# adamnelsonarcher/BB-OCR

Measured on AMD Instinct MI355X. Metric: book-page images/sec end-to-end (detect+recognize) @1280x960, higher is better.
Workload: dtype fp16

## Files before the change

### bb-ocr_amd/csrc/abi.cpp

```cpp
#include "ctx.h"

static hipError_t create_seq_stream(hipStream_t* s) {
    return hipStreamCreateWithFlags(s, hipStreamNonBlocking);
}

extern "C" {

void bbocr_default_params(bbocr_params* p) {
    if (!p) return;
    memset(p, 0, sizeof(*p));
    p->text_threshold = 0.7; p->low_text = 0.4; p->link_threshold = 0.4; p->canvas_size = 2560; p->mag_ratio = 1.0;
    p->slope_ths = 0.1; p->ycenter_ths = 0.5; p->height_ths = 0.5; p->width_ths = 0.5; p->add_margin = 0.1; p->min_size = 20;
    p->contrast_ths = 0.1; p->adjust_contrast = 0.5;
    p->decoder = BBOCR_DECODER_GREEDY; p->beam_width = 5;
}

int bbocr_create(const bbocr_config* cfg, bbocr_ctx** out) {
    if (!out) return BBOCR_ERR_ARG;
    *out = nullptr;
    bbocr_ctx* c = nullptr;
    try {
        c = new bbocr_ctx();
        c->root = c;
        if (cfg) c->cfg = *cfg;
        if (c->cfg.precision < BBOCR_PREC_BF16 || c->cfg.precision > BBOCR_PREC_EXACT_REC || c->cfg.call_slots < 0 || c->cfg.call_slots > kMaxSlots ||
            c->cfg.rec_quant < 0 || c->cfg.rec_quant > 1 || (c->cfg.rec_quant == 1 && !rec_split(c))) {
            delete c;
            return BBOCR_ERR_ARG;
        }
        int ndev = 0;
        if (hipGetDeviceCount(&ndev) != hipSuccess || ndev <= 0 || c->cfg.device < 0 || c->cfg.device >= ndev) {
            delete c;
            return BBOCR_ERR_HIP;
        }
        if (hipSetDevice(c->cfg.device) != hipSuccess || hipStreamCreateWithFlags(&c->stream, hipStreamNonBlocking) != hipSuccess ||
            hipStreamCreateWithFlags(&c->stream2, hipStreamNonBlocking) != hipSuccess ||
            create_seq_stream(&c->seq_stream) != hipSuccess ||
            hipMalloc(&c->zero_page, 256) != hipSuccess || hipMemset(c->zero_page, 0, 256) != hipSuccess) {
            delete c;
            return BBOCR_ERR_HIP;
        }
    } catch (...) {
        delete c;
        return BBOCR_ERR_INTERNAL;
    }
    c->cur = c->stream;
    *out = c;
    return BBOCR_OK;
}

}

bbocr_ctx* slot_create(bbocr_ctx* root) {
    bbocr_ctx* s = new bbocr_ctx();
    s->root = root;
    s->cfg = root->cfg;
    s->stream = root->stream;
    hipError_t e = hipStreamCreateWithFlags(&s->stream2, hipStreamNonBlocking);
    if (e == hipSuccess) e = create_seq_stream(&s->seq_stream);
    if (e != hipSuccess) {
        if (s->stream2) (void)hipStreamDestroy(s->stream2);
        delete s;
        fail(BBOCR_ERR_HIP, std::string("call slot: ") + hipGetErrorString(e));
    }
    s->cur = s->stream;
    return s;
}

void slot_destroy(bbocr_ctx* c) {
    if (c->stream2) (void)hipStreamSynchronize(c->stream2);
    if (c->seq_stream) (void)hipStreamSynchronize(c->seq_stream);
    if (c->feat_ev) (void)hipEventDestroy(c->feat_ev);
    for (hipEvent_t e : c->sub_events) (void)hipEventDestroy(e);
    if (c->det_t0) { (void)hipEventDestroy(c->det_t0); (void)hipEventDestroy(c->det_t1); }
    if (c->ccl_t0) { (void)hipEventDestroy(c->ccl_t0); (void)hipEventDestroy(c->ccl_t1); }
    if (c->sync_ev) (void)hipEventDestroy(c->sync_ev);
    if (c->seq_t1) { (void)hipEventDestroy(c->seq_t1); (void)hipEventDestroy(c->seq_t2); }
    for (auto& r : c->prof_recs) { (void)hipEventDestroy(r.e0); (void)hipEventDestroy(r.e1); }
    for (hipEvent_t e : c->prof_pool) (void)hipEventDestroy(e);
    DevBuf* bufs[] = {&c->arena.buf, &c->heat, &c->gray, &c->resized, &c->ccl_label, &c->ccl_stat, &c->ccl_slot, &c->ccl_comps, &c->ccl_rowext,
                      &c->ccl_counters, &c->crop_desc, &c->crop_desc2, &c->crop_scratch, &c->crop_hscratch, &c->crop_wscratch, &c->crop_luts, &c->crop_hist,
                      &c->ctc_idx, &c->ctc_pmax, &c->ctc_out_idx, &c->ctc_out, &c->seq_v, &c->seq_xp, &c->seq_h, &c->seq_lin, &c->seq_logits,
                      &c->seq_tables, &c->pp_gray, &c->pp_a, &c->pp_b, &c->pp_c, &c->pp_tab, &c->ctc_probs, &c->ctc_beam_idx, &c->ctc_beam_len, &c->ac_work, &c->th_coef, &c->je_scan, &c->je_out, &c->pe_out,
                      &c->pg_rgb, &c->pg_tab, &c->seq_q8, &c->seq_rowp};
    for (DevBuf* b : bufs) b->release();
    if (c->stream2) (void)hipStreamDestroy(c->stream2);
    if (c->seq_stream) (void)hipStreamDestroy(c->seq_stream);
    if (c->root != c) delete c;
}

namespace {
struct ThreadTimes { const bbocr_ctx* root = nullptr; float ms[8] = {0}; };
thread_local ThreadTimes tl_times;
thread_local std::string tl_err;
}
void publish_times(const bbocr_ctx* s) {
    tl_times.root = s->root;
    memcpy(tl_times.ms, s->times, sizeof(tl_times.ms));
}

extern "C" {

void bbocr_destroy(bbocr_ctx* c) {
    if (!c) return;
    (void)hipSetDevice(c->cfg.device);
    if (c->stream) (void)hipStreamSynchronize(c->stream);
    dist_release(c);
    for (bbocr_ctx* s : c->slots) slot_destroy(s);
    c->slots.clear();
    free_weights(c);
    slot_destroy(c);
    if (c->zero_page) (void)hipFree(c->zero_page);
    for (SideLane* l : {&c->upload_lane, &c->jpeg_lane})
        if (l->stream) (void)hipStreamDestroy(l->stream);
    if (c->stream) (void)hipStreamDestroy(c->stream);
    delete c;
}

const char* bbocr_last_error(bbocr_ctx* c) {
    if (!c) return "null context";
    std::lock_guard<std::mutex> lk(c->pool_mu);
    tl_err = c->err;
    return tl_err.c_str();
}

// ... 62 lines not shown
        detect_impl(ctx, dev_rgb, B, H, W, pp, dev_heat_out);
        slot_sync(ctx, ctx->stream);
        prof_collect(ctx);
        ctx->times[0] = ctx->times[7] = (float)ms_since(t0);
    });
}

int bbocr_boxes(bbocr_ctx* ctx, const float* dev_heat, int B, int h, int w, double ratio, const bbocr_params* p, bbocr_boxlist** out) {
    return guarded(ctx, [&](bbocr_ctx* ctx) {
        bbocr_params pp;
        bbocr_default_params(&pp);
        if (p) pp = *p;
        if (!dev_heat || !out) fail(BBOCR_ERR_ARG, "null pointer");
        memset(ctx->times, 0, sizeof(ctx->times));
        auto t0 = clk::now();
        HostBoxes hb;
        boxes_impl(ctx, dev_heat, B, h, w, ratio, pp, hb, ctx->stream);
        *out = export_boxes(hb);
        ctx->times[7] = (float)ms_since(t0);
    });
}

int bbocr_recognize(bbocr_ctx* ctx, const uint8_t* dev_gray, int B, int H, int W, const bbocr_boxlist* boxes, const bbocr_params* p,
                    bbocr_result** out) {
    return guarded(ctx, [&](bbocr_ctx* ctx) {
        bbocr_params pp;
        bbocr_default_params(&pp);
        if (p) pp = *p;
        if (!dev_gray || !boxes || !out || boxes->n_images != B) fail(BBOCR_ERR_ARG, "bad recognise arguments");
        memset(ctx->times, 0, sizeof(ctx->times));
        auto t0 = clk::now();
        HostBoxes hb;
        import_boxes(boxes, hb);
        std::vector<BoxJob> jobs;
        std::vector<int> off;
        recognize_impl(ctx, GrayPages{dev_gray, H, W}, B, hb, pp, jobs, off);
        prof_collect(ctx);
        *out = export_result(B, jobs, off);
        ctx->times[7] = (float)ms_since(t0);
    });
}

int bbocr_readtext_batch(bbocr_ctx* ctx, const uint8_t* dev_rgb, const uint8_t* dev_gray, int B, int H, int W, const bbocr_params* p,
                         bbocr_result** out) {
    return guarded(ctx, [&](bbocr_ctx* ctx) {
        bbocr_params pp;
        bbocr_default_params(&pp);
        if (p) pp = *p;
        if (!dev_rgb || !out) fail(BBOCR_ERR_ARG, "null pointer");
        memset(ctx->times, 0, sizeof(ctx->times));
        auto t_all = clk::now();
        const DetDims d = det_dims(H, W, pp.canvas_size, pp.mag_ratio);
        ctx->heat.ensure((size_t)B * d.h * d.w * 2 * sizeof(float));
        if (!dev_gray) {
            ctx->gray.ensure((size_t)B * H * W);
            HIPCHK(launch_gray(dev_rgb, (uint8_t*)ctx->gray.p, (size_t)B * H * W, ctx->stream));
            dev_gray = (const uint8_t*)ctx->gray.p;
        }
        std::vector<std::pair<int, int>> subs;
        if (!ctx->det_t0) { HIPCHK(hipEventCreate(&ctx->det_t0)); HIPCHK(hipEventCreate(&ctx->det_t1)); }
        HIPCHK(hipEventRecord(ctx->det_t0, ctx->stream));
        detect_impl(ctx, dev_rgb, B, H, W, pp, (float*)ctx->heat.p, [&](int b0, int nb) {
            if (subs.size() >= ctx->sub_events.size()) {
                hipEvent_t e;
                HIPCHK(hipEventCreateWithFlags(&e, hipEventDisableTiming));
                ctx->sub_events.push_back(e);
            }
            HIPCHK(hipEventRecord(ctx->sub_events[subs.size()], ctx->stream));
            subs.push_back({b0, nb});
        });
        HIPCHK(hipEventRecord(ctx->det_t1, ctx->stream));
        HostBoxes hb;
        hb.polys.resize(B); hb.hori.resize(B); hb.freeb.resize(B);
        RecEarly early;
        for (size_t k = 0; k < subs.size(); ++k) {
            const int b0 = subs[k].first, nb = subs[k].second;
            HIPCHK(hipStreamWaitEvent(ctx->stream2, ctx->sub_events[k], 0));
            HostBoxes part;
            boxes_impl(ctx, (const float*)ctx->heat.p + (size_t)b0 * d.h * d.w * 2, nb, d.h, d.w, d.ratio, pp, part, ctx->stream2);
            for (int i = 0; i < nb; ++i) {
                hb.polys[b0 + i] = std::move(part.polys[i]);
                hb.hori[b0 + i] = std::move(part.hori[i]);
                hb.freeb[b0 + i] = std::move(part.freeb[i]);
            }
            if (subs.size() >= 2 && k + 2 == subs.size() && pp.rotation_info[0] == 0 && ctx->crnn_loaded)
                rec_early_begin(ctx, GrayPages{dev_gray, H, W}, b0 + nb, B, hb, pp, early);
        }
        HIPCHK(hipEventSynchronize(ctx->det_t1));
        float det_ms = 0.f;
        HIPCHK(hipEventElapsedTime(&det_ms, ctx->det_t0, ctx->det_t1));
        ctx->times[0] = det_ms;
        std::vector<BoxJob> jobs;
        std::vector<int> off;
        recognize_impl(ctx, GrayPages{dev_gray, H, W}, B, hb, pp, jobs, off, &early);
        prof_collect(ctx);
        *out = export_result(B, jobs, off);
        ctx->times[7] = (float)ms_since(t_all);
    });
}

void bbocr_preproc_defaults(bbocr_preproc_params* p, int legacy) {
    if (!p) return;
    memset(p, 0, sizeof(*p));
    p->scale = 1.5; p->unsharp_radius = 1.0; p->unsharp_threshold = 3;
    if (legacy) { p->blur_sigma = 5.0; p->contrast = 1.3; p->brightness = 0.0; p->clahe_clip = 2.0; p->unsharp_percent = 20; }
    else        { p->blur_sigma = 3.0; p->contrast = 1.9; p->brightness = 1.2; p->clahe_clip = 2.5; p->unsharp_percent = 30; }
}

int bbocr_preprocess_chain(bbocr_ctx* ctx, const uint8_t* dev_bgr, int H, int W, const bbocr_preproc_params* p, uint8_t* dev_out, int* out_h,
                           int* out_w) {
    return guarded(ctx, [&](bbocr_ctx* ctx) {
        bbocr_preproc_params q;
        bbocr_preproc_defaults(&q, 0);
        if (p) q = *p;
        if (H <= 0 || W <= 0) fail(BBOCR_ERR_ARG, "bad image shape");
        if (q.scale < 0 || q.blur_sigma < 0 || q.contrast < 0 || q.brightness < 0 || q.clahe_clip < 0 || q.unsharp_radius < 0 || q.unsharp_percent < 0)
            fail(BBOCR_ERR_ARG, "negative pre-processing parameter");
        const int dh = q.scale > 0 ? (int)(H * q.scale) : H, dw = q.scale > 0 ? (int)(W * q.scale) : W;
        if (out_h) *out_h = dh;
        if (out_w) *out_w = dw;
        if (!dev_out) return;
        if (!dev_bgr) fail(BBOCR_ERR_ARG, "null device pointer");
        if (dh <= 0 || dw <= 0) fail(BBOCR_ERR_ARG, "image collapses to zero size");
        if (q.clahe_clip > 0 && (dh < 16 || dw < 16)) fail(BBOCR_ERR_ARG, "image too small for the 8x8 CLAHE tile grid");
        preprocess_chain_impl(ctx, dev_bgr, H, W, q, dev_out, dh, dw);
    });
}

int bbocr_preprocess_book_cover(bbocr_ctx* ctx, const uint8_t* dev_bgr, int H, int W, uint8_t* dev_out, int* out_h, int* out_w) {
    bbocr_preproc_params q;
    bbocr_preproc_defaults(&q, 0);
    return bbocr_preprocess_chain(ctx, dev_bgr, H, W, &q, dev_out, out_h, out_w);
}

void bbocr_free_boxlist(bbocr_boxlist* b) {
    if (!b) return;
    free(b->poly_off); free(b->polys); free(b->hori_off); free(b->hori); free(b->free_off); free(b->free_q);
    free(b);
}

void bbocr_free_result(bbocr_result* r) {
    if (!r) return;
    free(r->box_off); free(r->quads); free(r->is_free); free(r->text_off); free(r->text_idx); free(r->conf);
    free(r);
}

int bbocr_set_profiling(bbocr_ctx* ctx, int on) {
// ... 25 lines not shown
```

### bb-ocr_amd/csrc/ctx.h

```cpp
#pragma once
#include "../../include/bbocr.h"

#include <algorithm>
#include <atomic>
#include <chrono>
#include <condition_variable>
#include <cmath>
#include <cstring>
#include <functional>
#include <map>
#include <memory>
#include <mutex>
#include <string>
#include <thread>
#include <unordered_map>
#include <vector>

#include "boxpost.h"
#include "hostpool.h"
#include "common.h"
#include "kernels.h"


using clk = std::chrono::steady_clock;
// ... 112 lines not shown
    bool craft_loaded = false;
    uint16_t* c11_wf = nullptr;
    float* c11_b = nullptr;
    float* c11_w32 = nullptr;
    float* cls6_w32 = nullptr;
    ConvPlan conv1_2, conv2_1, conv2_2, conv3_1, conv3_2, conv3_3, conv4_1, conv4_2, conv4_3, conv5_1, conv5_2, fc6, fc7;
    ConvPlan up1a, up1b, up2b, up3b, up4b, cls0, cls2, cls4;
    ConvPlan up2y, up2s, up3y, up3s, up4y, up4s;
    float* cls_tail = nullptr;
    uint16_t* cls_tail_frag = nullptr;
    uint16_t* up4y_post = nullptr;
    bool crnn_loaded = false;
    float* r0_wb = nullptr;
    uint16_t* r0_afrag = nullptr;
    ConvPlan r1, r2, r3, r4, r5, r6, xproj[2], lin[2], pred;
    uint16_t* whh[2] = {nullptr, nullptr};
    float whh_scale[2] = {1.f, 1.f};
    struct Q8Layer { int8_t* w = nullptr; float* scale = nullptr; float* bias = nullptr; };
    Q8Layer q_ih[2], q_hh[2], q_lin[2], q_pred;
    void* zero_page = nullptr;
};

struct bbocr_ctx : WeightView {
    bbocr_config cfg{};
    bbocr_ctx* root = nullptr;
    std::vector<bbocr_ctx*> slots;
    std::mutex pool_mu;
    std::condition_variable pool_cv;
    std::mutex enq_mu;
    ConvRoute op_conv_route{};
    bool slot_busy = false;
    hipStream_t stream = nullptr;
    DevBuf pp_gray, pp_a, pp_b, pp_c, pp_tab;
    DevBuf ac_work;
    DevBuf th_coef;
    int th_coef_key[6] = {0, 0, 0, 0, 0, 0};
    int th_coef_ks[2] = {0, 0};
    int th_coef_rows[2] = {0, 0};
    DevBuf je_scan, je_out;
    DevBuf pe_out;
    DevBuf pp_cubic;
    int pp_cubic_key[4] = {0, 0, 0, 0};
    unsigned long long pp_cubic_K[2] = {0, 0};
    unsigned int ignore_mask[4] = {0, 0, 0, 0};
    int beam_width = 0;
    hipStream_t cur = nullptr;
    SideLane upload_lane;
    SideLane jpeg_lane;
    PinBuf jd_pin;
    DevBuf jd_in, jd_work, jd_coef, jd_stage;
    DevBuf jd_page;
    long long jd_count[4] = {0, 0, 0, 0};
    hipStream_t seq_stream = nullptr;
    hipEvent_t feat_ev = nullptr;
    hipStream_t stream2 = nullptr;
    std::vector<hipEvent_t> sub_events;
    hipEvent_t ccl_t0 = nullptr, ccl_t1 = nullptr;
    hipEvent_t det_t0 = nullptr, det_t1 = nullptr;
    hipEvent_t sync_ev = nullptr;
    hipEvent_t seq_t1 = nullptr, seq_t2 = nullptr;
    std::string err;
    float times[8] = {0};

    struct ProfRec { hipEvent_t e0, e1; double flops; int group; };
    int profiling = 0;
    int prof_group = 0;
    std::vector<ProfRec> prof_recs;
    std::vector<hipEvent_t> prof_pool;
    double prof_ms[2] = {0, 0}, prof_flops[2] = {0, 0};
    long long prof_launches[2] = {0, 0};

    void* dist_comm = nullptr;
    int dist_rank = 0, dist_world = 0;
    std::unique_ptr<HostPool> pool;
    std::vector<void*> owned;
    std::vector<size_t> owned_bytes;

    Arena arena;
    DevBuf heat, gray, resized;
    DevBuf pg_rgb, pg_tab;
    PinBuf pg_pin;
    DevBuf ccl_label, ccl_stat, ccl_slot, ccl_comps, ccl_rowext, ccl_counters;
    DevBuf crop_desc, crop_scratch, crop_hscratch, crop_wscratch, crop_luts, crop_hist;
    DevBuf ctc_idx, ctc_pmax, ctc_out_idx, ctc_out, ctc_probs, ctc_beam_idx, ctc_beam_len, crop_desc2;
    PinBuf desc_pin, desc_pin2;
    PinBuf ctc_pin;
    DevBuf seq_v, seq_xp, seq_h, seq_lin, seq_logits, seq_tables;
    DevBuf seq_q8, seq_rowp;
};

inline int det_el(const bbocr_ctx* c) { return (c->cfg.precision == BBOCR_PREC_FP16 || c->cfg.precision == BBOCR_PREC_EXACT || c->cfg.precision == BBOCR_PREC_EXACT_REC) ? 1 : 0; }
inline int rec_el(const bbocr_ctx* c) { return c->cfg.precision != BBOCR_PREC_BF16 ? 1 : 0; }
inline bool rec_split(const bbocr_ctx* c) { return c->cfg.precision == BBOCR_PREC_EXACT || c->cfg.precision == BBOCR_PREC_EXACT_REC; }
inline bool rec_quant(const bbocr_ctx* c) { return c->cfg.rec_quant == 1; }
inline bool det_split(const bbocr_ctx* c) { return c->cfg.precision == BBOCR_PREC_EXACT; }

struct TensorMap {
    std::unordered_map<std::string, const bbocr_tensor_desc*> m;
    bool zeros = false;
    std::vector<float> zero_buf;
    TensorMap() : zeros(true), zero_buf((size_t)5 << 20, 0.f) {}
    TensorMap(const bbocr_tensor_desc* d, int n) {
        for (int i = 0; i < n; ++i) {
            std::string k = d[i].name ? d[i].name : "";
            if (k.rfind("module.", 0) == 0) k = k.substr(7);
            m[k] = &d[i];
        }
// ... 160 lines not shown
void crnn_seq_xproj(bbocr_ctx* c, int l, const uint16_t* x, size_t rows_pad, void* xp);
void crnn_seq_xproj_conv(bbocr_ctx* c, int l, const uint16_t* x, size_t rows_pad, void* xp);
void crnn_seq_lin(bbocr_ctx* c, int l, const uint16_t* h, size_t rows_pad, uint16_t* out);
void crnn_seq_pred(bbocr_ctx* c, const uint16_t* x, size_t rows_pad, float* logits);
void rec_seq_tiles(const bbocr_ctx* c, RecRun& run);
enum { CTC_GREEDY = 0, CTC_BEAM_HOST = 1, CTC_BEAM_DEVICE = 2 };
int ctc_route(int beam_width, int C, const int* seqs, int nseq);
void ctc_size(bbocr_ctx* c, size_t rows, int nseq, int cs, int route);
double ctc_decode(const CtcOut& o, const int* idx, int n, std::vector<int>& text);
void rec_early_begin(bbocr_ctx* c, const GrayPages& g, int pages, int B, const HostBoxes& hb, const bbocr_params& p, RecEarly& e);
void recognize_impl(bbocr_ctx* c, const GrayPages& g, int B, const HostBoxes& hb, const bbocr_params& p, std::vector<BoxJob>& jobs, std::vector<int>& box_off, RecEarly* early = nullptr);
bbocr_result* export_result(int B, const std::vector<BoxJob>& jobs, const std::vector<int>& box_off);
void pp_resize(bbocr_ctx* c, const uint8_t* src, int H, int W, uint8_t* dst, int dh, int dw, bool src_bgr = false);
void pp_gauss(bbocr_ctx* c, const uint8_t* src, int H, int W, uint8_t* dst, double sigma);
const uint8_t* pp_fold_lut(bbocr_ctx* c, size_t n, double contrast, double brightness);
void pp_clahe(bbocr_ctx* c, const uint8_t* src, int H, int W, const uint8_t* d_lut, uint8_t* dst, double clip_limit);
void pp_unsharp(bbocr_ctx* c, const uint8_t* src, int H, int W, uint8_t* dst, uint8_t* tmp1, uint8_t* tmp2, float radius, int percent, int threshold);
void preprocess_chain_impl(bbocr_ctx* c, const uint8_t* bgr, int H, int W, const bbocr_preproc_params& q, uint8_t* out, int dh, int dw);
void gaussian_taps_fixed(int n, double sigma, int* k);

inline HostPool& host_pool(bbocr_ctx* c) {
    if (!c->pool) {
        const int want = c->cfg.host_threads > 0 ? c->cfg.host_threads : std::min(16, host_cpu_share());
        c->pool.reset(new HostPool(std::max(1, std::min(want, 64)) - 1));
    }
    return *c->pool;
}

inline bool other_call_in_flight(bbocr_ctx* c) {
    bbocr_ctx* root = c->root;
    std::lock_guard<std::mutex> lk(root->pool_mu);
    if (root != c && root->slot_busy) return true;
    for (bbocr_ctx* s : root->slots)
        if (s != c && s->slot_busy) return true;
    return false;
}

struct EnqLock {
    std::unique_lock<std::mutex> lk;
    explicit EnqLock(bbocr_ctx* c) : lk(c->root->enq_mu) {}
};
constexpr int kMaxSlots = 2;
bbocr_ctx* slot_create(bbocr_ctx* root);
void slot_destroy(bbocr_ctx* s);
void publish_times(const bbocr_ctx* s);
void dist_release(bbocr_ctx* root);

inline void slot_sync(bbocr_ctx* c, hipStream_t st) {
    if (!c->sync_ev) HIPCHK(hipEventCreateWithFlags(&c->sync_ev, hipEventDisableTiming));
    HIPCHK(hipEventRecord(c->sync_ev, st));
    HIPCHK(hipEventSynchronize(c->sync_ev));
}

inline void prof_release(bbocr_ctx* c, const bbocr_ctx::ProfRec& r) { c->prof_pool.push_back(r.e0); c->prof_pool.push_back(r.e1); }

inline void guarded_drain(bbocr_ctx* ctx) {
    if (ctx->stream) (void)hipStreamSynchronize(ctx->stream);
    if (ctx->stream2) (void)hipStreamSynchronize(ctx->stream2);
    if (ctx->seq_stream) (void)hipStreamSynchronize(ctx->seq_stream);
    ctx->cur = ctx->stream;
    (void)hipGetLastError();
    for (auto& r : ctx->prof_recs) prof_release(ctx, r);
    ctx->prof_recs.clear();
}

struct SlotLease {
    bbocr_ctx* root;
    bbocr_ctx* slot = nullptr;
    bool exclusive;
    SlotLease(bbocr_ctx* r, bool excl) : root(r), exclusive(excl) {
        std::unique_lock<std::mutex> lk(root->pool_mu);
        const int max_slots = root->cfg.call_slots == 1 ? 1 : kMaxSlots;
        if (exclusive) {
            root->pool_cv.wait(lk, [&] {
                if (root->slot_busy) return false;
                for (bbocr_ctx* s : root->slots) if (s->slot_busy) return false;
                return true;
            });
            root->slot_busy = true;
            for (bbocr_ctx* s : root->slots) s->slot_busy = true;
            slot = root;
            return;
        }
        for (;;) {
            if (!root->slot_busy) { slot = root; break; }
            for (bbocr_ctx* s : root->slots) if (!s->slot_busy) { slot = s; break; }
            if (slot) break;
            if ((int)root->slots.size() + 1 < max_slots) {
                slot = slot_create(root);
                root->slots.push_back(slot);
                break;
            }
            root->pool_cv.wait(lk);
        }
        slot->slot_busy = true;
        if (slot != root) {
            static_cast<WeightView&>(*slot) = static_cast<const WeightView&>(*root);
            slot->cfg = root->cfg;
            slot->profiling = root->profiling;
        }
    }
    ~SlotLease() {
        {
            std::lock_guard<std::mutex> lk(root->pool_mu);
            if (exclusive) {
                root->slot_busy = false;
// ... 65 lines not shown
```

### bb-ocr_amd/csrc/recognizer.cpp

```cpp
#include "ctx.h"

void crop_refit_fw(CropDesc& d) {
    const int cw = (int)std::ceil(64 * ((double)d.rw / (double)d.rh));
    d.fw = cw > d.imgW ? d.imgW : cw;
}

static bool plan_sizes(CropDesc& d, int width, int height) {
    double ratio = (double)width / (double)height;
    if (ratio < 1.0) {
        ratio = 1.0 / ratio;
        d.rw = 64; d.rh = (int)(64 * ratio);
    } else {
        d.rw = (int)(64 * ratio); d.rh = 64;
    }
    if ((int)(64 * ratio) == 0) return false;
    d.imgW = (int)std::ceil(std::max(ratio, 1.0)) * 64;
    crop_refit_fw(d);
    return d.rw > 0 && d.rh > 0 && d.fw > 0;
}

bool plan_horizontal(const std::array<int, 4>& box, int img, int H, int W, BoxJob& j) {
    const int x_min = std::max(0, box[0]), x_max = std::min(box[1], W), y_min = std::max(0, box[2]), y_max = std::min(box[3], H);
    const int width = x_max - x_min, height = y_max - y_min;
    if (width <= 0 || height <= 0) return false;
// ... 137 lines not shown

static Act seq_rows(const bbocr_ctx* c, const uint16_t* p, size_t rows_pad, int C) { return Act{(uint16_t*)p, 1, (int)(rows_pad / 256), 256, C * rec_mul(c)}; }
void crnn_seq_xproj_conv(bbocr_ctx* c, int l, const uint16_t* x, size_t rows_pad, void* xp) {
    run_conv(c, c->xproj[l], seq_rows(c, x, rows_pad, 256), false, nullptr, false, false, xp, 2048, 2048, rec_split(c));
}
void crnn_seq_xproj(bbocr_ctx* c, int l, const uint16_t* x, size_t rows_pad, void* xp) {
    if (!rec_split(c)) {
        if (c->arena.dry) return;
        if (launch_seq_proj_profiled(c, c->xproj[l], x, rows_pad, (uint16_t*)xp) == hipSuccess) return;
    }
    crnn_seq_xproj_conv(c, l, x, rows_pad, xp);
}
void crnn_seq_lin(bbocr_ctx* c, int l, const uint16_t* h, size_t rows_pad, uint16_t* out) {
    run_conv(c, c->lin[l], seq_rows(c, h, rows_pad, 512), false, nullptr, false, false, out, 256 * rec_mul(c), 256, false);
}
void crnn_seq_pred(bbocr_ctx* c, const uint16_t* x, size_t rows_pad, float* logits) {
    run_conv(c, c->pred, seq_rows(c, x, rows_pad, 256), false, nullptr, false, false, logits, 112, 112, true);
}

static size_t rec_max_rows(const bbocr_ctx* c) { return c->cfg.rec_max_cols > 0 ? (size_t)std::max(64, c->cfg.rec_max_cols / 4) : (size_t)1500000; }

void rec_plan_part(const std::vector<BoxJob>& jobs, const std::vector<int>& sel, int res0, size_t row_base, RecPart& part) {
    std::map<int, std::vector<int>> buckets;
    for (size_t k = 0; k < sel.size(); ++k) buckets[jobs[sel[k]].d.imgW].push_back((int)k);
    size_t rows = row_base, cols = 0;
    for (auto& kv : buckets) {
        const int imgW = kv.first, T = imgW / 4 - 1;
        RecChunk ch{imgW, T, (int)part.descs.size(), (int)kv.second.size(), rows};
        for (int i = 0; i < ch.n; ++i) {
            const int k = kv.second[i];
            CropDesc d = jobs[sel[k]].d;
            if (cols > 0x7ff00000u) fail(BBOCR_ERR_OVERFLOW, "recogniser pass wider than 2^31 columns");
            d.slot = (int)cols;
            d.pad_ = (int)(rows + (size_t)i * T);
            cols += (size_t)imgW + REC_GAP;
            part.any_warp |= d.warp != 0;
            part.any_tall |= !(d.fw == d.rw && d.rh == 64);
            part.descs.push_back(d);
            part.order.push_back(res0 + k);
        }
        rows += (size_t)ch.n * T;
        part.chunks.push_back(ch);
    }
    part.rows = rows - row_base;
    part.cols = cols;
}

const CropDesc* rec_upload_descs(bbocr_ctx* c, const RecPart& part, DevBuf& desc_buf) {
    const size_t bytes = part.descs.size() * sizeof(CropDesc);
    desc_buf.ensure(bytes);
    PinBuf& pin = (&desc_buf == &c->crop_desc2) ? c->desc_pin2 : c->desc_pin;
    pin.ensure(bytes);
    memcpy(pin.p, part.descs.data(), bytes);
    HIPCHK(hipMemcpyAsync(desc_buf.p, pin.p, bytes, hipMemcpyHostToDevice, c->stream));
    return (const CropDesc*)desc_buf.p;
}

uint16_t* rec_wide_image(bbocr_ctx* c, const RecPart& part) {
    c->arena.begin(true);
    (void)c->arena.alloc<uint16_t>((size_t)64 * part.cols);
    crnn_features_wide(c, part, nullptr, nullptr);
    c->arena.buf.ensure(c->arena.off);
    c->arena.begin(false);
    return c->arena.alloc<uint16_t>((size_t)64 * part.cols);
}

void rec_launch_crops(bbocr_ctx* c, const GrayPages& g, const RecPart& part, const CropDesc* dd, uint16_t* wide, int stage) {
    const int n = (int)part.descs.size(), Wt = (int)part.cols;
    HIPCHK(launch_crops(g.gray, g.H, g.W, dd, 0, n, 0, part.any_warp, part.any_tall, (uint8_t*)c->crop_wscratch.p, (uint8_t*)c->crop_scratch.p,
                        (uint8_t*)c->crop_hscratch.p, (const uint8_t*)c->crop_luts.p, wide, stage, c->stream, wide ? Wt : 0, wide ? REC_GAP : 0,
                        wide ? rec_mode(c) : 0, g.tab_dev));
}

static void rec_launch_part(bbocr_ctx* c, const GrayPages& g, const RecPart& part, DevBuf& desc_buf, bool stage_a) {
    if (part.descs.empty()) return;
    EnqLock enq(c);
    const CropDesc* dd = rec_upload_descs(c, part, desc_buf);
    if (stage_a) rec_launch_crops(c, g, part, dd, nullptr, 1);
    uint16_t* wide = rec_wide_image(c, part);
    rec_launch_crops(c, g, part, dd, wide, 2);
    crnn_features_wide(c, part, dd, wide);
    if (!c->feat_ev) HIPCHK(hipEventCreateWithFlags(&c->feat_ev, hipEventDisableTiming));
    HIPCHK(hipEventRecord(c->feat_ev, c->stream));
}

void rec_add_tables(RecRun& run, const RecPart& part, int tile_seqs) {
    for (const RecChunk& ch : part.chunks) {
        for (int s0 = 0; s0 < ch.n; s0 += tile_seqs) {
            run.tiles.push_back((int)(ch.row0 + (size_t)s0 * ch.T));
            run.tiles.push_back(std::min(tile_seqs, ch.n - s0));
            run.tiles.push_back(ch.T);
            run.tiles.push_back(0);
        }
        for (int i = 0; i < ch.n; ++i) {
            run.seqs.push_back((int)(ch.row0 + (size_t)i * ch.T));
            run.seqs.push_back(ch.T);
            run.seq_k.push_back(part.order[ch.first + i]);
        }
    }
    run.rows += part.rows;
}

int ctc_route(int beam_width, int C, const int* seqs, int nseq) {
    if (beam_width <= 0) return CTC_GREEDY;
    int max_T = 0;
    for (int i = 0; i < nseq; ++i) max_T = std::max(max_T, seqs[2 * i + 1]);
    return ctc_beam_on_device(beam_width, C, max_T) ? CTC_BEAM_DEVICE : CTC_BEAM_HOST;
}

void ctc_size(bbocr_ctx* c, size_t rows, int nseq, int cs, int route) {
    c->ctc_idx.ensure(rows * 4);
    c->ctc_pmax.ensure(rows * 4);
    c->ctc_out_idx.ensure(rows * 4);
    c->ctc_out.ensure((size_t)nseq * sizeof(CtcOut));
    if (route != CTC_GREEDY) c->ctc_probs.ensure(rows * cs * sizeof(float));
    if (route == CTC_BEAM_DEVICE) {
        c->ctc_beam_idx.ensure(rows * 4);
        c->ctc_beam_len.ensure((size_t)nseq * 4);
    }
}

double ctc_decode(const CtcOut& o, const int* idx, int n, std::vector<int>& text) {
    text.assign(idx, idx + n);
    return o.cnt > 0 ? std::pow((double)o.prod, 2.0 / std::sqrt((double)o.cnt)) : 0.0;
}

static void rec_finish(bbocr_ctx* c, RecRun& run, std::vector<std::vector<int>>& texts, std::vector<double>& confs) {
    const size_t rows = run.rows;
    if (rows == 0) return;
    const size_t rows_pad = align_up(rows, 256);
    auto t0 = clk::now();
    rec_seq_tiles(c, run);
    {
        std::vector<int>& tiles = run.tiles;
        const size_t nt = tiles.size() / 4;
        std::vector<size_t> perm(nt);
        for (size_t i = 0; i < nt; ++i) perm[i] = i;
        std::stable_sort(perm.begin(), perm.end(), [&](size_t x, size_t y) { return tiles[x * 4 + 2] > tiles[y * 4 + 2]; });
        std::vector<int> t2(tiles.size());
        for (size_t i = 0; i < nt; ++i) memcpy(&t2[i * 4], &tiles[perm[i] * 4], 16);
        tiles.swap(t2);
    }
    const std::vector<int>&tiles = run.tiles, &seqs = run.seqs;
    const int ntiles = (int)(tiles.size() / 4), nseq = (int)(seqs.size() / 2);
    c->seq_logits.ensure(rows_pad * 112 * 4);
    c->seq_tables.ensure((tiles.size() + seqs.size()) * 4);
    int* tiles_dev = (int*)c->seq_tables.p;
    int* seqs_dev = tiles_dev + tiles.size();
    const int route = ctc_route(c->beam_width, 97, seqs.data(), nseq);
    ctc_size(c, rows, nseq, 112, route);
    const size_t oo_off = align_up(rows * 4, 16);
    const size_t bi_off = align_up(oo_off + (size_t)nseq * sizeof(CtcOut), 16), bl_off = bi_off + align_up(rows * 4, 16);
    c->ctc_pin.ensure(route == CTC_BEAM_DEVICE ? bl_off + (size_t)nseq * 4 : bi_off);
    const int* oidx = (const int*)c->ctc_pin.p;
    const CtcOut* oo = (const CtcOut*)((const char*)c->ctc_pin.p + oo_off);
    const int* bidx = (const int*)((const char*)c->ctc_pin.p + bi_off);
    const int* blen = (const int*)((const char*)c->ctc_pin.p + bl_off);
    std::vector<float> probs(route == CTC_BEAM_HOST ? rows * 112 : 0);
    std::vector<std::vector<int>> beam_texts;
    if (!c->seq_t1) { HIPCHK(hipEventCreate(&c->seq_t1)); HIPCHK(hipEventCreate(&c->seq_t2)); }
    {
        hipStream_t ss = (c->seq_stream && c->feat_ev) ? c->seq_stream : c->stream;
        std::unique_lock<std::mutex> enq;
        if (ss == c->stream) enq = std::unique_lock<std::mutex>(c->root->enq_mu);
        else HIPCHK(hipStreamWaitEvent(ss, c->feat_ev, 0));
        c->cur = ss;
        struct Restore { bbocr_ctx* c; ~Restore() { c->cur = c->stream; } } restore{c};
        HIPCHK(hipMemcpyAsync(tiles_dev, tiles.data(), tiles.size() * 4, hipMemcpyHostToDevice, ss));
        HIPCHK(hipMemcpyAsync(seqs_dev, seqs.data(), seqs.size() * 4, hipMemcpyHostToDevice, ss));
        crnn_sequence(c, rows, rows_pad, tiles_dev, ntiles, seqs_dev, nseq, (float*)c->seq_logits.p);
        HIPCHK(hipEventRecord(c->seq_t1, ss));
        HIPCHK(launch_ctc((const float*)c->seq_logits.p, rows, 97, 112, seqs_dev, nseq, (int*)c->ctc_idx.p, (float*)c->ctc_pmax.p,
                          (int*)c->ctc_out_idx.p, (CtcOut*)c->ctc_out.p, ss, c->ignore_mask, route != CTC_GREEDY ? (float*)c->ctc_probs.p : nullptr));
        if (route != CTC_BEAM_DEVICE) HIPCHK(hipMemcpyAsync(c->ctc_pin.p, c->ctc_out_idx.p, rows * 4, hipMemcpyDeviceToHost, ss));
        HIPCHK(hipMemcpyAsync((char*)c->ctc_pin.p + oo_off, c->ctc_out.p, (size_t)nseq * sizeof(CtcOut), hipMemcpyDeviceToHost, ss));
        if (route == CTC_BEAM_DEVICE) {
            int max_T = 0;
            for (int i = 0; i < nseq; ++i) max_T = std::max(max_T, seqs[2 * i + 1]);
            HIPCHK(launch_ctc_beam((const float*)c->ctc_probs.p, rows, 97, 112, seqs_dev, nseq, max_T, c->beam_width, (int*)c->ctc_beam_idx.p,
                                   (int*)c->ctc_beam_len.p, ss));
            HIPCHK(hipMemcpyAsync((char*)c->ctc_pin.p + bi_off, c->ctc_beam_idx.p, rows * 4, hipMemcpyDeviceToHost, ss));
            HIPCHK(hipMemcpyAsync((char*)c->ctc_pin.p + bl_off, c->ctc_beam_len.p, (size_t)nseq * 4, hipMemcpyDeviceToHost, ss));
        } else if (route == CTC_BEAM_HOST) {
            HIPCHK(hipMemcpyAsync(probs.data(), c->ctc_probs.p, probs.size() * sizeof(float), hipMemcpyDeviceToHost, ss));
        }
        HIPCHK(hipEventRecord(c->seq_t2, ss));
    }
    HIPCHK(hipEventSynchronize(c->seq_t2));
    float ctc_ms = 0.f;
    HIPCHK(hipEventElapsedTime(&ctc_ms, c->seq_t1, c->seq_t2));
    c->times[4] += (float)ms_since(t0) - ctc_ms;
    c->times[5] += ctc_ms;
    t0 = clk::now();
    if (route == CTC_BEAM_HOST) ctc_beam_search_batch(probs.data(), seqs.data(), nseq, 97, 112, c->beam_width, beam_texts, &host_pool(c));
    for (int i = 0; i < nseq; ++i) {
        const int k = run.seq_k[i];
        if (route == CTC_BEAM_HOST) confs[k] = ctc_decode(oo[i], beam_texts[i].data(), (int)beam_texts[i].size(), texts[k]);
        else if (route == CTC_BEAM_DEVICE) confs[k] = ctc_decode(oo[i], bidx + seqs[2 * i], std::clamp(blen[i], 0, seqs[2 * i + 1]), texts[k]);
        else confs[k] = ctc_decode(oo[i], oidx + seqs[2 * i], oo[i].len, texts[k]);
    }
    c->times[5] += (float)ms_since(t0);
}

static std::vector<std::vector<int>> rec_split_runs(const bbocr_ctx* c, const std::vector<BoxJob>& jobs, const std::vector<int>& sel) {
    std::vector<int> byw(sel.size());
    for (size_t k = 0; k < sel.size(); ++k) byw[k] = (int)k;
    std::stable_sort(byw.begin(), byw.end(), [&](int x, int y) { return jobs[sel[x]].d.imgW < jobs[sel[y]].d.imgW; });
    std::vector<std::vector<int>> runs(1);
    size_t rows = 0;
    for (int k : byw) {
        const size_t t = (size_t)(jobs[sel[k]].d.imgW / 4 - 1);
        if (!runs.back().empty() && rows + t > rec_max_rows(c)) { runs.emplace_back(); rows = 0; }
        runs.back().push_back(k);
        rows += t;
    }
    return runs;
}

static void recognise_pass(bbocr_ctx* c, const GrayPages& g, std::vector<BoxJob>& jobs, const std::vector<int>& sel,
                           bool stage_a, std::vector<std::vector<int>>& texts, std::vector<double>& confs) {
// ... 1 lines not shown
    confs.assign(sel.size(), 0.0);
    if (sel.empty()) return;
    for (const std::vector<int>& ks : rec_split_runs(c, jobs, sel)) {
        std::vector<int> sub(ks.size());
        for (size_t i = 0; i < ks.size(); ++i) sub[i] = sel[ks[i]];
        RecPart part;
        rec_plan_part(jobs, sub, 0, 0, part);
        for (size_t i = 0; i < part.order.size(); ++i) part.order[i] = ks[part.order[i]];
        auto t0 = clk::now();
        c->seq_v.ensure(align_up(part.rows, 256) * 256 * 2 * rec_mul(c));
        rec_launch_part(c, g, part, c->crop_desc, stage_a);
        c->times[3] += (float)ms_since(t0);
        RecRun run;
        rec_add_tables(run, part, lstm_tile_seqs(rec_mode(c)));
        rec_finish(c, run, texts, confs);
    }
}

static double percentile_u8(const unsigned int* hist, size_t n, double q) {
    const double virt = (double)(n - 1) * (q / 100.0);
    const double prev = std::floor(virt);
    const double gamma = virt - prev;
    const size_t i0 = (size_t)prev, i1 = std::min(i0 + 1, n - 1);
    auto at = [&](size_t idx) {
        size_t acc = 0;
        for (int v = 0; v < 256; ++v) {
            acc += hist[v];
            if (idx < acc) return v;
        }
        return 255;
    };
    const int a = at(i0), b = at(i1);
    const double diff = (double)(b - a);
    double r = (double)a + diff * gamma;
    if (gamma >= 0.5) r = (double)b - diff * (1 - gamma);
    return r;
}

bool contrast_lut(const unsigned int* hist, size_t npx, double target, uint8_t* lut) {
    const double high = percentile_u8(hist, npx, 90.0), lowp = percentile_u8(hist, npx, 10.0);
    const double contrast = (high - lowp) / std::max(10.0, high + lowp);
    if (!(contrast < target)) return false;
    const double ratio = 200.0 / std::max(10.0, high - lowp);
    for (int v = 0; v < 256; ++v) {
        double x = ((double)v - lowp + 25) * ratio;
        x = std::max(0.0, std::min(255.0, x));
        lut[v] = (uint8_t)x;
    }
    return true;
}

std::vector<int> crop_contrast_luts(bbocr_ctx* c, const CropDesc* descs_dev, std::vector<CropDesc>& descs, double target, std::vector<uint8_t>& luts) {
    c->crop_hist.ensure(descs.size() * 256 * 4);
    HIPCHK(launch_crop_hist((const uint8_t*)c->crop_scratch.p, descs_dev, 0, (int)descs.size(), (unsigned int*)c->crop_hist.p, c->stream));
    std::vector<unsigned int> hist(descs.size() * 256);
    HIPCHK(hipMemcpyAsync(hist.data(), c->crop_hist.p, hist.size() * 4, hipMemcpyDeviceToHost, c->stream));
    slot_sync(c, c->stream);
    std::vector<int> changed;
    for (size_t k = 0; k < descs.size(); ++k) {
        uint8_t lut[256];
        if (!contrast_lut(&hist[k * 256], (size_t)descs[k].rw * descs[k].rh, target, lut)) continue;
        descs[k].lut_off = (int)luts.size();
        luts.insert(luts.end(), lut, lut + 256);
        changed.push_back((int)k);
    }
    return changed;
}

static void rec_check_params(bbocr_ctx* c, const bbocr_params& p) {
    if (!c->crnn_loaded) fail(BBOCR_ERR_STATE, "recogniser weights not loaded");
    if (p.ignore_mask[0] & 1u) fail(BBOCR_ERR_ARG, "the CTC blank (class 0) cannot be ignored");
    for (int i = 0; i < 4; ++i) c->ignore_mask[i] = p.ignore_mask[i];
    if (p.decoder != BBOCR_DECODER_GREEDY && p.decoder != BBOCR_DECODER_BEAMSEARCH) fail(BBOCR_ERR_ARG, "unknown decoder");
    if (p.decoder == BBOCR_DECODER_BEAMSEARCH && p.beam_width <= 0) fail(BBOCR_ERR_ARG, "beam_width must be positive");
    c->beam_width = p.decoder == BBOCR_DECODER_BEAMSEARCH ? p.beam_width : 0;
}

static void rec_plan_pages(const HostBoxes& hb, int b0, int b1, const GrayPages& g, std::vector<BoxJob>& jobs, std::vector<int>& box_off) {
    for (int b = b0; b < b1; ++b) {
        for (const auto& hbx : hb.hori[b]) {
            BoxJob j;
            if (plan_horizontal(hbx, b, g.h(b), g.w(b), j)) jobs.push_back(j);
        }
        for (const auto& fq : hb.freeb[b]) {
            BoxJob j;
            if (plan_free(fq, b, j)) jobs.push_back(j);
        }
        box_off[b + 1] = (int)jobs.size();
    }
}

void rec_layout_scratch(std::vector<BoxJob>& jobs, size_t first, size_t& a_total, size_t& w_total) {
    for (size_t i = first; i < jobs.size(); ++i) {
        BoxJob& j = jobs[i];
        j.d.a_off = (int)a_total;
        a_total += align_up((size_t)j.d.rw * j.d.rh, 16);
        if (j.d.warp) {
            j.d.warp_off = (int)w_total;
            w_total += align_up((size_t)j.d.sw * j.d.sh, 16);
        }
        if (a_total > 0x7fffffff || w_total > 0x7fffffff) fail(BBOCR_ERR_OVERFLOW, "crop scratch exceeds 2 GiB");
    }
}

void rec_early_begin(bbocr_ctx* c, const GrayPages& g, int pages, int B, const HostBoxes& hb, const bbocr_params& p, RecEarly& e) {
    rec_check_params(c, p);
    e.box_off.assign(pages + 1, 0);
    rec_plan_pages(hb, 0, pages, g, e.jobs, e.box_off);
    if (e.jobs.empty()) return;
    rec_layout_scratch(e.jobs, 0, e.a_total, e.w_total);
// ... 82 lines not shown
    } collapse{jobs, n_base, nrot};
    if (jobs.empty()) return;
    std::vector<std::vector<int>> texts;
    std::vector<double> confs;
    if (resume) {
        size_t a_total = early->a_total, w_total = early->w_total;
        rec_layout_scratch(jobs, n_early, a_total, w_total);
        c->crop_scratch.ensure_keep(std::max<size_t>(a_total, 16), early->a_total);
        c->crop_hscratch.ensure_keep(std::max<size_t>(a_total, 16), 0);
        c->crop_wscratch.ensure_keep(std::max<size_t>(w_total, 16), 0);
        texts.assign(jobs.size(), {});
        confs.assign(jobs.size(), 0.0);
        std::vector<int> rest(jobs.size() - n_early);
        for (size_t i = 0; i < rest.size(); ++i) rest[i] = (int)(n_early + i);
        RecPart part2;
        rec_plan_part(jobs, rest, (int)n_early, early->part.rows, part2);
        RecRun run;
        rec_add_tables(run, early->part, lstm_tile_seqs(rec_mode(c)));
        if (early->part.rows + part2.rows <= rec_max_rows(c)) {
            c->seq_v.ensure_keep(align_up(early->part.rows + part2.rows, 256) * 256 * 2 * rec_mul(c), early->part.rows * 256 * 2 * rec_mul(c));
            auto t0 = clk::now();
            rec_launch_part(c, g, part2, c->crop_desc2, true);
            c->times[3] += (float)ms_since(t0);
            rec_add_tables(run, part2, lstm_tile_seqs(rec_mode(c)));
            rec_finish(c, run, texts, confs);
        } else {
            rec_finish(c, run, texts, confs);
            std::vector<std::vector<int>> t2;
            std::vector<double> c2;
            recognise_pass(c, g, jobs, rest, true, t2, c2);
            for (size_t i = 0; i < rest.size(); ++i) { texts[rest[i]] = t2[i]; confs[rest[i]] = c2[i]; }
        }
        early->active = false;
    } else {
        size_t a_total = 0, w_total = 0;
        rec_layout_scratch(jobs, 0, a_total, w_total);
        c->crop_scratch.ensure(std::max<size_t>(a_total, 16));
        c->crop_hscratch.ensure(std::max<size_t>(a_total, 16));
        c->crop_wscratch.ensure(std::max<size_t>(w_total, 16));
        c->crop_luts.ensure(256);
        std::vector<int> all(jobs.size());
        for (size_t i = 0; i < jobs.size(); ++i) all[i] = (int)i;
        recognise_pass(c, g, jobs, all, true, texts, confs);
    }
    for (size_t i = 0; i < jobs.size(); ++i) { jobs[i].text = texts[i]; jobs[i].conf = confs[i]; }
    std::vector<int> low;
    for (size_t i = 0; i < jobs.size(); ++i)
        if (jobs[i].conf < p.contrast_ths) low.push_back((int)i);
    if (low.empty() || !(p.adjust_contrast > 0)) return;
    auto t0 = clk::now();
    std::vector<CropDesc> ld(low.size());
    for (size_t k = 0; k < low.size(); ++k) ld[k] = jobs[low[k]].d;
    c->crop_desc.ensure(ld.size() * sizeof(CropDesc));
    HIPCHK(hipMemcpyAsync(c->crop_desc.p, ld.data(), ld.size() * sizeof(CropDesc), hipMemcpyHostToDevice, c->stream));
    std::vector<int> redo;
    std::vector<uint8_t> luts;
    for (int k : crop_contrast_luts(c, (const CropDesc*)c->crop_desc.p, ld, p.adjust_contrast, luts)) {
        jobs[low[k]].d.lut_off = ld[k].lut_off;
        redo.push_back(low[k]);
    }
    if (!redo.empty()) {
        c->crop_luts.ensure(luts.size());
        HIPCHK(hipMemcpyAsync(c->crop_luts.p, luts.data(), luts.size(), hipMemcpyHostToDevice, c->stream));
        std::vector<std::vector<int>> t2;
        std::vector<double> c2;
        recognise_pass(c, g, jobs, redo, false, t2, c2);
        for (size_t k = 0; k < redo.size(); ++k) {
            BoxJob& j = jobs[redo[k]];
            j.d.lut_off = -1;
            if (!(j.conf > c2[k])) { j.text = t2[k]; j.conf = c2[k]; }
        }
    }
    c->times[6] += (float)ms_since(t0);
}

bbocr_result* export_result(int B, const std::vector<BoxJob>& jobs, const std::vector<int>& box_off) {
    bbocr_result* r = (bbocr_result*)calloc(1, sizeof(bbocr_result));
    const size_t nb = jobs.size();
    r->n_images = B;
    r->box_off = (int*)calloc(B + 1, sizeof(int));
    for (int b = 0; b <= B; ++b) r->box_off[b] = box_off[b];
    r->quads = (double*)calloc(std::max<size_t>(1, nb) * 8, sizeof(double));
    r->is_free = (int*)calloc(std::max<size_t>(1, nb), sizeof(int));
    r->text_off = (int*)calloc(nb + 1, sizeof(int));
    r->conf = (double*)calloc(std::max<size_t>(1, nb), sizeof(double));
    size_t nt = 0;
    for (const BoxJob& j : jobs) nt += j.text.size();
    r->text_idx = (int*)calloc(std::max<size_t>(1, nt), sizeof(int));
    size_t o = 0;
    for (size_t i = 0; i < nb; ++i) {
        memcpy(r->quads + i * 8, jobs[i].quad, 64);
        r->is_free[i] = jobs[i].is_free;
        r->conf[i] = jobs[i].conf;
        r->text_off[i] = (int)o;
        for (int v : jobs[i].text) r->text_idx[o++] = v;
    }
    r->text_off[nb] = (int)o;
    return r;
}
```

Before: 993.5.

## Split recogniser front-end and final stage onto side streams around shared main stream

Recogniser part launches now run crop extraction and the first CRNN stage on a side stream, and only the middle stages on the shared main stream under the enqueue lock. The last stage goes to the sequence stream, ordered by new front/gather events. Gray conversion and the contrast-retry pass are also moved to the front stream. The aim is to overlap crop and feature work with detection and other callers on the main stream and to shorten lock hold time, at the cost of extra cross-stream events and more complex ordering.

Measured after the change: 998.1, median of 6. Within noise of the previous version (+0.5%).

```diff
diff --git a/bb-ocr_amd/csrc/abi.cpp b/bb-ocr_amd/csrc/abi.cpp
--- a/bb-ocr_amd/csrc/abi.cpp
+++ b/bb-ocr_amd/csrc/abi.cpp
@@ -71,6 +71,8 @@
     if (c->stream2) (void)hipStreamSynchronize(c->stream2);
     if (c->seq_stream) (void)hipStreamSynchronize(c->seq_stream);
     if (c->feat_ev) (void)hipEventDestroy(c->feat_ev);
+    if (c->front_ev) (void)hipEventDestroy(c->front_ev);
+    if (c->gath_ev) (void)hipEventDestroy(c->gath_ev);
     for (hipEvent_t e : c->sub_events) (void)hipEventDestroy(e);
     if (c->det_t0) { (void)hipEventDestroy(c->det_t0); (void)hipEventDestroy(c->det_t1); }
     if (c->ccl_t0) { (void)hipEventDestroy(c->ccl_t0); (void)hipEventDestroy(c->ccl_t1); }
@@ -239,9 +241,10 @@
         auto t_all = clk::now();
         const DetDims d = det_dims(H, W, pp.canvas_size, pp.mag_ratio);
         ctx->heat.ensure((size_t)B * d.h * d.w * 2 * sizeof(float));
-        if (!dev_gray) {
+        const bool own_gray = !dev_gray;
+        if (own_gray) {
             ctx->gray.ensure((size_t)B * H * W);
-            HIPCHK(launch_gray(dev_rgb, (uint8_t*)ctx->gray.p, (size_t)B * H * W, ctx->stream));
+            HIPCHK(launch_gray(dev_rgb, (uint8_t*)ctx->gray.p, (size_t)B * H * W, front_stream(ctx)));
             dev_gray = (const uint8_t*)ctx->gray.p;
         }
         std::vector<std::pair<int, int>> subs;
@@ -280,6 +283,7 @@
         std::vector<BoxJob> jobs;
         std::vector<int> off;
         recognize_impl(ctx, GrayPages{dev_gray, H, W}, B, hb, pp, jobs, off, &early);
+        if (own_gray) slot_sync(ctx, front_stream(ctx));
         prof_collect(ctx);
         *out = export_result(B, jobs, off);
         ctx->times[7] = (float)ms_since(t_all);
diff --git a/bb-ocr_amd/csrc/ctx.h b/bb-ocr_amd/csrc/ctx.h
--- a/bb-ocr_amd/csrc/ctx.h
+++ b/bb-ocr_amd/csrc/ctx.h
@@ -188,7 +188,9 @@
     DevBuf jd_page;
     long long jd_count[4] = {0, 0, 0, 0};
     hipStream_t seq_stream = nullptr;
+    hipEvent_t front_ev = nullptr;
     hipEvent_t feat_ev = nullptr;
+    hipEvent_t gath_ev = nullptr;
     hipStream_t stream2 = nullptr;
     std::vector<hipEvent_t> sub_events;
     hipEvent_t ccl_t0 = nullptr, ccl_t1 = nullptr;
@@ -455,6 +457,15 @@
     HIPCHK(hipEventSynchronize(c->sync_ev));
 }
 
+inline bool side_streams(const bbocr_ctx* c) { return c->stream2 && c->seq_stream; }
+inline hipStream_t front_stream(const bbocr_ctx* c) { return side_streams(c) ? c->stream2 : c->stream; }
+inline hipStream_t seq_stream_of(const bbocr_ctx* c) { return side_streams(c) ? c->seq_stream : c->stream; }
+struct CurStream {
+    bbocr_ctx* c;
+    CurStream(bbocr_ctx* ctx, hipStream_t s) : c(ctx) { c->cur = s; }
+    ~CurStream() { c->cur = c->stream; }
+};
+
 inline void prof_release(bbocr_ctx* c, const bbocr_ctx::ProfRec& r) { c->prof_pool.push_back(r.e0); c->prof_pool.push_back(r.e1); }
 
 inline void guarded_drain(bbocr_ctx* ctx) {
diff --git a/bb-ocr_amd/csrc/recognizer.cpp b/bb-ocr_amd/csrc/recognizer.cpp
--- a/bb-ocr_amd/csrc/recognizer.cpp
+++ b/bb-ocr_amd/csrc/recognizer.cpp
@@ -213,7 +213,7 @@
     PinBuf& pin = (&desc_buf == &c->crop_desc2) ? c->desc_pin2 : c->desc_pin;
     pin.ensure(bytes);
     memcpy(pin.p, part.descs.data(), bytes);
-    HIPCHK(hipMemcpyAsync(desc_buf.p, pin.p, bytes, hipMemcpyHostToDevice, c->stream));
+    HIPCHK(hipMemcpyAsync(desc_buf.p, pin.p, bytes, hipMemcpyHostToDevice, c->cur));
     return (const CropDesc*)desc_buf.p;
 }
 
@@ -229,20 +229,43 @@
 void rec_launch_crops(bbocr_ctx* c, const GrayPages& g, const RecPart& part, const CropDesc* dd, uint16_t* wide, int stage) {
     const int n = (int)part.descs.size(), Wt = (int)part.cols;
     HIPCHK(launch_crops(g.gray, g.H, g.W, dd, 0, n, 0, part.any_warp, part.any_tall, (uint8_t*)c->crop_wscratch.p, (uint8_t*)c->crop_scratch.p,
-                        (uint8_t*)c->crop_hscratch.p, (const uint8_t*)c->crop_luts.p, wide, stage, c->stream, wide ? Wt : 0, wide ? REC_GAP : 0,
+                        (uint8_t*)c->crop_hscratch.p, (const uint8_t*)c->crop_luts.p, wide, stage, c->cur, wide ? Wt : 0, wide ? REC_GAP : 0,
                         wide ? rec_mode(c) : 0, g.tab_dev));
 }
 
 static void rec_launch_part(bbocr_ctx* c, const GrayPages& g, const RecPart& part, DevBuf& desc_buf, bool stage_a) {
     if (part.descs.empty()) return;
-    EnqLock enq(c);
+    const bool side = side_streams(c);
+    hipStream_t fs = front_stream(c), gs = seq_stream_of(c);
+    for (hipEvent_t* e : {&c->feat_ev, &c->front_ev, &c->gath_ev})
+        if (!*e) HIPCHK(hipEventCreateWithFlags(e, hipEventDisableTiming));
+    std::unique_lock<std::mutex> enq;
+    if (!side) enq = std::unique_lock<std::mutex>(c->root->enq_mu);
+    CurStream cur(c, fs);
+    if (side) {
+        if (c->det_t1) HIPCHK(hipStreamWaitEvent(fs, c->det_t1, 0));
+        HIPCHK(hipStreamWaitEvent(fs, c->gath_ev, 0));
+    }
     const CropDesc* dd = rec_upload_descs(c, part, desc_buf);
     if (stage_a) rec_launch_crops(c, g, part, dd, nullptr, 1);
     uint16_t* wide = rec_wide_image(c, part);
     rec_launch_crops(c, g, part, dd, wide, 2);
-    crnn_features_wide(c, part, dd, wide);
-    if (!c->feat_ev) HIPCHK(hipEventCreateWithFlags(&c->feat_ev, hipEventDisableTiming));
+    Act a = crnn_features_stages(c, part, dd, Act{wide, 1, 64, (int)part.cols, 1}, 0, 0);
+    if (side) {
+        HIPCHK(hipEventRecord(c->front_ev, fs));
+        enq = std::unique_lock<std::mutex>(c->root->enq_mu);
+        HIPCHK(hipStreamWaitEvent(c->stream, c->front_ev, 0));
+    }
+    c->cur = c->stream;
+    a = crnn_features_stages(c, part, dd, a, 1, REC_STAGES - 2);
     HIPCHK(hipEventRecord(c->feat_ev, c->stream));
+    if (side) {
+        enq.unlock();
+        HIPCHK(hipStreamWaitEvent(gs, c->feat_ev, 0));
+    }
+    c->cur = gs;
+    (void)crnn_features_stages(c, part, dd, a, REC_STAGES - 1, REC_STAGES - 1);
+    if (side) HIPCHK(hipEventRecord(c->gath_ev, gs));
 }
 
 void rec_add_tables(RecRun& run, const RecPart& part, int tile_seqs) {
@@ -321,12 +344,10 @@
     std::vector<std::vector<int>> beam_texts;
     if (!c->seq_t1) { HIPCHK(hipEventCreate(&c->seq_t1)); HIPCHK(hipEventCreate(&c->seq_t2)); }
     {
-        hipStream_t ss = (c->seq_stream && c->feat_ev) ? c->seq_stream : c->stream;
+        hipStream_t ss = seq_stream_of(c);
         std::unique_lock<std::mutex> enq;
         if (ss == c->stream) enq = std::unique_lock<std::mutex>(c->root->enq_mu);
-        else HIPCHK(hipStreamWaitEvent(ss, c->feat_ev, 0));
-        c->cur = ss;
-        struct Restore { bbocr_ctx* c; ~Restore() { c->cur = c->stream; } } restore{c};
+        CurStream cur(c, ss);
         HIPCHK(hipMemcpyAsync(tiles_dev, tiles.data(), tiles.size() * 4, hipMemcpyHostToDevice, ss));
         HIPCHK(hipMemcpyAsync(seqs_dev, seqs.data(), seqs.size() * 4, hipMemcpyHostToDevice, ss));
         crnn_sequence(c, rows, rows_pad, tiles_dev, ntiles, seqs_dev, nseq, (float*)c->seq_logits.p);
@@ -434,10 +455,10 @@
 
 std::vector<int> crop_contrast_luts(bbocr_ctx* c, const CropDesc* descs_dev, std::vector<CropDesc>& descs, double target, std::vector<uint8_t>& luts) {
     c->crop_hist.ensure(descs.size() * 256 * 4);
-    HIPCHK(launch_crop_hist((const uint8_t*)c->crop_scratch.p, descs_dev, 0, (int)descs.size(), (unsigned int*)c->crop_hist.p, c->stream));
+    HIPCHK(launch_crop_hist((const uint8_t*)c->crop_scratch.p, descs_dev, 0, (int)descs.size(), (unsigned int*)c->crop_hist.p, c->cur));
     std::vector<unsigned int> hist(descs.size() * 256);
-    HIPCHK(hipMemcpyAsync(hist.data(), c->crop_hist.p, hist.size() * 4, hipMemcpyDeviceToHost, c->stream));
-    slot_sync(c, c->stream);
+    HIPCHK(hipMemcpyAsync(hist.data(), c->crop_hist.p, hist.size() * 4, hipMemcpyDeviceToHost, c->cur));
+    slot_sync(c, c->cur);
     std::vector<int> changed;
     for (size_t k = 0; k < descs.size(); ++k) {
         uint8_t lut[256];
@@ -626,16 +647,17 @@
     std::vector<CropDesc> ld(low.size());
     for (size_t k = 0; k < low.size(); ++k) ld[k] = jobs[low[k]].d;
     c->crop_desc.ensure(ld.size() * sizeof(CropDesc));
-    HIPCHK(hipMemcpyAsync(c->crop_desc.p, ld.data(), ld.size() * sizeof(CropDesc), hipMemcpyHostToDevice, c->stream));
     std::vector<int> redo;
     std::vector<uint8_t> luts;
+    CurStream cur(c, front_stream(c));
+    HIPCHK(hipMemcpyAsync(c->crop_desc.p, ld.data(), ld.size() * sizeof(CropDesc), hipMemcpyHostToDevice, c->cur));
     for (int k : crop_contrast_luts(c, (const CropDesc*)c->crop_desc.p, ld, p.adjust_contrast, luts)) {
         jobs[low[k]].d.lut_off = ld[k].lut_off;
         redo.push_back(low[k]);
     }
     if (!redo.empty()) {
         c->crop_luts.ensure(luts.size());
-        HIPCHK(hipMemcpyAsync(c->crop_luts.p, luts.data(), luts.size(), hipMemcpyHostToDevice, c->stream));
+        HIPCHK(hipMemcpyAsync(c->crop_luts.p, luts.data(), luts.size(), hipMemcpyHostToDevice, c->cur));
         std::vector<std::vector<int>> t2;
         std::vector<double> c2;
         recognise_pass(c, g, jobs, redo, false, t2, c2);
```
